# jdhuang-csm/hybrid-drt

Measured on AMD Instinct MI355X. Metric: DRT fits/sec (256 freq x 512 tau, batched), higher is better.
Workload: dtype f64

## Files before the change

hybrid-drt_amd/csrc/gram.hip:

```cpp
#include "common.hpp"
#include <type_traits>

namespace hipdrt {

typedef double v4d __attribute__((ext_vector_type(4)));

static constexpr int GT = 64;
static constexpr int GK = 16;
static constexpr int GLD = 80;


__host__ __device__ inline bool gram_strip_folds(int n) { const int nt16 = (n + 15) >> 4; return (nt16 & 3) == 1 && nt16 > 1; }

struct GramSub { int r, c; };
__host__ __device__ constexpr GramSub gram_diag_sub(int e) {
    const int r = e >= 10 ? 4 : e >= 6 ? 3 : e >= 3 ? 2 : e >= 1 ? 1 : 0;
    return GramSub{r, e >= 14 ? 4 : e >= 10 ? e - 10 : e - r * (r + 1) / 2};
}

template <int TURN>
__device__ __forceinline__ void gram_diag_slab(const double* sl, v4d (&acc)[4], int needm) {
#pragma unroll
    for (int kk = 0; kk < GK; kk += 4) {
        double x[5];
#pragma unroll
        for (int c = 0; c < 5; ++c) x[c] = sl[kk * GLD + c * 16];
#pragma unroll
        for (int s = 0; s < 4; ++s) {
            const GramSub sub = gram_diag_sub(TURN + 4 * s);
            if (needm & (1 << s)) acc[s] = __builtin_amdgcn_mfma_f64_16x16x4f64(x[sub.c], x[sub.r], acc[s], 0, 0, 0);
        }
    }
}

template <bool DOP, bool ROWP>
__global__ __launch_bounds__(256, 5) void gram_kernel(int m, int n, const double* __restrict__ A, int lda,
                                                   const double* __restrict__ w, GramL2 g, double* __restrict__ P,
                                                   int ldp, long long p_stride, const int* __restrict__ active,
                                                   int ntile, double* __restrict__ Ppk, long long ppk_stride, int nchp,
                                                   long long a_stride) {
    const int b = blockIdx.y;
    if (active && !active[b]) return;
    A += (size_t)b * a_stride;
    int t = blockIdx.x, ti = 0;
    while (t >= ti + 1) { t -= ti + 1; ++ti; }
    const int tj = t;
    const int i0 = ti * GT, j0 = tj * GT;
    const bool diag = (ti == tj);
    const int nt16 = (n + 15) >> 4;
    const bool strip = diag && gram_strip_folds(n);
    const int s0 = (nt16 - 1) * 16;
    const bool last = strip && i0 + GT == s0;

    __shared__ double sI[GK * GLD];
    __shared__ double sJ[GK * GLD];

    const int tid = threadIdx.x, lane = tid & 63, wv = __builtin_amdgcn_readfirstlane(tid >> 6);
    const double* wb = w + (size_t)b * m;
    double* Pk = Ppk ? Ppk + (size_t)b * ppk_stride : nullptr;

    int nown = 0, needm = 0;
    const int turn = (wv + 2 * (ti & 1)) & 3;
    if (diag) {
        const int rows_all = (Pk && nchp > nt16 ? nchp : nt16) - 4 * ti, rows_data = nt16 - 4 * ti;
        const int nr = rows_all < 4 ? rows_all : 4, nd = rows_data < 4 ? rows_data : 4;
        nown = nr * (nr + 1) / 2 + (strip ? 4 : 0) + (last ? 1 : 0);
        const int nneed = strip ? nown : nd * (nd + 1) / 2;
#pragma unroll
        for (int s = 0; s < 4; ++s) needm |= (turn + 4 * s < nneed) << s;
    }
    const int qr = 4 * ti + 2 * (wv >> 1), qc = 4 * tj + 2 * (wv & 1);
    const bool need00 = qr < nt16 && qc < nt16, need01 = qr < nt16 && qc + 1 < nt16;
    const bool need10 = qr + 1 < nt16 && qc < nt16, need11 = qr + 1 < nt16 && qc + 1 < nt16;

    v4d acc[4];
#pragma unroll
    for (int s = 0; s < 4; ++s) acc[s] = (v4d){0.0, 0.0, 0.0, 0.0};

    const int sk = tid >> 4, sc = (tid & 15) * 4;
    const bool vec2 = ((lda | n) & 1) == 0 && (reinterpret_cast<size_t>(A) & 15) == 0;
    const bool full = vec2 && m >= GK && (m & (GK - 1)) == 0 && i0 + GT <= n && (diag || j0 + GT <= n);
    const bool smask = strip && s0 + (tid & 15) < n;
    double vi[4], vj[4], wkr = 0.0;
    const double *pI = nullptr, *pJ = nullptr;
    auto fetch = [&](auto DIAG, auto FORM, int k0) {
        constexpr bool D = decltype(DIAG)::value;
        constexpr int F = decltype(FORM)::value;
        if constexpr (F == 0) {
            wkr = wb[k0 + sk];
            const double2 t0 = *reinterpret_cast<const double2*>(pI), t1 = *reinterpret_cast<const double2*>(pI + 2);
            vi[0] = t0.x; vi[1] = t0.y; vi[2] = t1.x; vi[3] = t1.y;
            if constexpr (!D) {
                const double2 u0 = *reinterpret_cast<const double2*>(pJ), u1 = *reinterpret_cast<const double2*>(pJ + 2);
                vj[0] = u0.x; vj[1] = u0.y; vj[2] = u1.x; vj[3] = u1.y;
            } else if (strip) {
                vj[0] = *pJ;
            }
            pI += (size_t)GK * lda;
            pJ += (size_t)GK * lda;
        } else {
            const int k = k0 + sk;
#pragma unroll
            for (int e = 0; e < 4; ++e) { vi[e] = 0.0; vj[e] = 0.0; }
            wkr = 0.0;
            if (k < m) {
                wkr = wb[k];
                const double* row = A + (size_t)k * lda;
                if constexpr (F == 1) {
#pragma unroll
                    for (int e = 0; e < 4; e += 2) {
                        const int ci = i0 + sc + e, cj = j0 + sc + e;
                        if (ci < n) { const double2 t = *reinterpret_cast<const double2*>(row + ci); vi[e] = t.x; vi[e + 1] = t.y; }
                        if (!D && cj < n) { const double2 t = *reinterpret_cast<const double2*>(row + cj); vj[e] = t.x; vj[e + 1] = t.y; }
                    }
                } else {
#pragma unroll
                    for (int e = 0; e < 4; ++e) {
                        const int ci = i0 + sc + e, cj = j0 + sc + e;
                        if (ci < n) vi[e] = row[ci];
                        if (!D && cj < n) vj[e] = row[cj];
                    }
                }
                if (D && smask) vj[0] = row[s0 + (tid & 15)];
            }
        }
    };
    auto kloop = [&](auto DIAG, auto TURN, auto FORM) {
        constexpr bool D = decltype(DIAG)::value;
        constexpr bool FULL = decltype(FORM)::value == 0;
        if constexpr (FULL) {
            pI = A + (size_t)sk * lda + i0 + sc;
            pJ = A + (size_t)sk * lda + (D ? (smask ? s0 + (tid & 15) : n - 1) : j0 + sc);
        }
        fetch(DIAG, FORM, 0);
        for (int k0 = 0; k0 < m; k0 += GK) {
            __syncthreads();
            *reinterpret_cast<double2*>(&sI[sk * GLD + sc]) = make_double2(wkr * vi[0], wkr * vi[1]);
            *reinterpret_cast<double2*>(&sI[sk * GLD + sc + 2]) = make_double2(wkr * vi[2], wkr * vi[3]);
            if (!D) {
                *reinterpret_cast<double2*>(&sJ[sk * GLD + sc]) = make_double2(wkr * vj[0], wkr * vj[1]);
                *reinterpret_cast<double2*>(&sJ[sk * GLD + sc + 2]) = make_double2(wkr * vj[2], wkr * vj[3]);
            } else if (strip) {
                sI[sk * GLD + GT + (tid & 15)] = wkr * (FULL && !smask ? 0.0 : vj[0]);
            }
            __syncthreads();
            if (k0 + GK < m) fetch(DIAG, FORM, k0 + GK);
            if (!D) {
                const int wi = (wv >> 1) * 32, wj = (wv & 1) * 32;
#pragma unroll
                for (int kk = 0; kk < GK; kk += 4) {
                    const int kr = kk + (lane >> 4);
                    double a0 = sI[kr * GLD + wi + (lane & 15)];
                    double a1 = sI[kr * GLD + wi + 16 + (lane & 15)];
                    double b0 = sJ[kr * GLD + wj + (lane & 15)];
                    double b1 = sJ[kr * GLD + wj + 16 + (lane & 15)];
                    if (FULL || need00) acc[0] = __builtin_amdgcn_mfma_f64_16x16x4f64(b0, a0, acc[0], 0, 0, 0);
                    if (FULL || need01) acc[1] = __builtin_amdgcn_mfma_f64_16x16x4f64(b1, a0, acc[1], 0, 0, 0);
                    if (FULL || need10) acc[2] = __builtin_amdgcn_mfma_f64_16x16x4f64(b0, a1, acc[2], 0, 0, 0);
                    if (FULL || need11) acc[3] = __builtin_amdgcn_mfma_f64_16x16x4f64(b1, a1, acc[3], 0, 0, 0);
                }
            } else {
                const double* sl = sI + (lane >> 4) * GLD + (lane & 15);
                gram_diag_slab<decltype(TURN)::value>(sl, acc, needm);
            }
        }
    };
    auto kform = [&](auto DIAG, auto TURN) {
        if (full) kloop(DIAG, TURN, std::integral_constant<int, 0>{});
        else if (vec2) kloop(DIAG, TURN, std::integral_constant<int, 1>{});
        else kloop(DIAG, TURN, std::integral_constant<int, 2>{});
    };
    if (!diag) kform(std::false_type{}, std::integral_constant<int, 0>{});
    else if (turn == 0) kform(std::true_type{}, std::integral_constant<int, 0>{});
    else if (turn == 1) kform(std::true_type{}, std::integral_constant<int, 1>{});
    else if (turn == 2) kform(std::true_type{}, std::integral_constant<int, 2>{});
    else kform(std::true_type{}, std::integral_constant<int, 3>{});

    double* sqI = sI;
    double* sqJ = sJ;
    constexpr int TW = 2 * GT;
    double* tw = sI + 3 * GT;
    const int dbase = i0 - j0 - (GT - 1);
    constexpr int SW = GT + 16;
    double* sqS = sJ + 3 * GT;
    double* tws = sJ + 4 * GT;
    const int dbase_s = s0 - j0 - (GT - 1);
    double fac[3] = {0, 0, 0};
    const bool reach_known = !DOP && g.toep && g.toep_maxd >= 0 && (j0 >= g.ns || g.spec_zero);
    const bool l2on = g.s && !(reach_known && i0 >= g.ns && dbase > g.toep_maxd);
    const bool l2on_s = strip && g.s && !(reach_known && s0 >= g.ns && dbase_s > g.toep_maxd);
    if (l2on) {
#pragma unroll
        for (int k = 0; k < 3; ++k) fac[k] = g.dfac[k] * (g.use_rho ? g.rho[(size_t)b * 3 + k] : 1.0);
        __syncthreads();
        const double* sb_ = g.s + (size_t)b * 3 * n;
        for (int e = tid; e < 3 * GT; e += 256) {
            const int k = e / GT, c = e % GT;
            sqI[e] = (i0 + c < n) ? sqrt(sb_[k * n + i0 + c]) : 0.0;
            sqJ[e] = (j0 + c < n) ? sqrt(sb_[k * n + j0 + c]) : 0.0;
        }
        if (strip && tid < 3 * 16) {
            const int k = tid >> 4, c = tid & 15;
            sqS[tid] = (s0 + c < n) ? sqrt(sb_[k * n + s0 + c]) : 0.0;
        }
        if (g.toep) {
            const int nd = n - g.ns;
            for (int e = tid; e < 3 * TW; e += 256) {
                const int k = e / TW, sl = e % TW;
                int dd = dbase + sl;
                dd = dd < 0 ? -dd : dd;
                tw[e] = (g.dfac[k] > 0.0 && dd < nd) ? g.mk[k][(size_t)g.ns * g.ldm + g.ns + dd] * fac[k] : 0.0;
            }
            if (l2on_s && tid < 3 * SW) {
                const int k = tid / SW, dd = dbase_s + tid % SW;
                tws[tid] = (g.dfac[k] > 0.0 && dd < nd) ? g.mk[k][(size_t)g.ns * g.ldm + g.ns + dd] * fac[k] : 0.0;
            }
        }
        __syncthreads();
    }
    double* Pb = (ROWP && P) ? P + (size_t)b * p_stride : nullptr;
    double dfac2[3] = {0, 0, 0};
    if (l2on) {
        if (DOP) {
#pragma unroll
            for (int k = 0; k < 3; ++k) dfac2[k] = g.dop_dfac[k] * (g.use_rho ? g.dop_rho[(size_t)b * 3 + k] : 1.0);
        }
    }
    const int dop_lo = DOP ? g.dop_start : 0, dop_hi = DOP ? g.dop_start + g.dop_size : 0;
#pragma unroll
    for (int s = 0; s < 4; ++s) {
        int r16 = qr + (s >> 1), c16 = qc + (s & 1);
        bool srow = false, scol = false;
        if (diag) {
            const int e = turn + 4 * s;
            if (e >= nown) continue;
            const GramSub sub = gram_diag_sub(e);
            srow = sub.r == 4;
            scol = sub.c == 4;
            r16 = srow ? nt16 - 1 : 4 * ti + sub.r;
            c16 = scol ? nt16 - 1 : 4 * ti + sub.c;
        }
        const bool sw = srow && !scol;
        const bool on = sw ? l2on_s : l2on;
        const double* sqr = srow ? sqS - s0 : sqI - i0;
        const double* sqc = scol ? sqS - s0 : sqJ - j0;
        const int rstr = srow ? 16 : GT, cstr = scol ? 16 : GT;
        const double* win = sw ? tws - dbase_s : tw - dbase;
        const int wstr = sw ? SW : TW;
        double vals[4];
#pragma unroll
        for (int r = 0; r < 4; ++r) {
            const int i = r16 * 16 + (lane & 15);
            const int j = c16 * 16 + (lane >> 4) + 4 * r;
            double v = 0.0;
            if (i < n && j < n) {
                v = acc[s][r];
                if (on) {
                    double l2 = 0.0;
#pragma unroll
                    for (int k = 0; k < 3; ++k) {
                        if (g.dfac[k] > 0.0) {
                            double mv;
                            if (g.toep && i >= g.ns && j >= g.ns) {
                                mv = win[k * wstr + (i - j)];
                            } else {
                                mv = g.sym ? g.mk[k][(size_t)j * g.ldm + i] : g.mk[k][(size_t)i * g.ldm + j];
                                if (i >= g.ns && j >= g.ns) mv *= fac[k];
                                else if (DOP && i >= dop_lo && i < dop_hi && j >= dop_lo && j < dop_hi) mv *= dfac2[k];
                            }
                            l2 += (sqr[k * rstr + i] * mv) * sqc[k * cstr + j];
                        }
                    }
                    v += l2;
                } else if (!g.s && g.l2) {
                    v += g.l2[(size_t)b * g.l2_stride + (size_t)i * g.ldl2 + j];
                }
                if (ROWP && Pb && j <= i) {
                    Pb[(size_t)i * ldp + j] = v;
                    if (i != j) Pb[(size_t)j * ldp + i] = v;
                }
            }
            vals[r] = v;
        }
        if (Pk && r16 < nchp && c16 < nchp && r16 >= c16) {
            double2* tile = reinterpret_cast<double2*>(Pk + ((size_t)r16 * nchp + c16) * 256);
            const int fo = (lane & 15) * 4 + (lane >> 4);
            tile[fo] = make_double2(vals[0], vals[1]);
            tile[64 + fo] = make_double2(vals[2], vals[3]);
        }
    }
    if (Pk && strip) {
        const int pe = nchp < nt16 + 3 ? nchp : nt16 + 3;
        for (int pr = nt16; pr < pe; ++pr) {
#pragma unroll
            for (int h = 0; h < 2; ++h) {
                const int pc = h ? nt16 - 1 + wv : 4 * ti + wv;
                if (h && !(last && pc <= pr)) continue;
                double2* tile = reinterpret_cast<double2*>(Pk + ((size_t)pr * nchp + pc) * 256);
                tile[lane] = make_double2(0.0, 0.0);
                tile[64 + lane] = make_double2(0.0, 0.0);
            }
        }
    }
}

__global__ __launch_bounds__(64) void pack_p_kernel(int n, const double* __restrict__ P, int ldp, long long p_stride,
                                                    double* __restrict__ Ppk, long long ppk_stride, int nchp) {
    int t = blockIdx.x, tr = 0;
    while (t >= tr + 1) { t -= tr + 1; ++tr; }
    const int tc = t, b = blockIdx.y, lane = threadIdx.x;
    const double* Pb = P + (size_t)b * p_stride;
    double vals[4];
#pragma unroll
    for (int r = 0; r < 4; ++r) {
        const int i = tr * 16 + (lane & 15), j = tc * 16 + (lane >> 4) + 4 * r;
        double v = 0.0;
        if (i < n && j < n) v = (i >= j) ? Pb[(size_t)i * ldp + j] : Pb[(size_t)j * ldp + i];
        vals[r] = v;
    }
    double2* tile = reinterpret_cast<double2*>(Ppk + (size_t)b * ppk_stride + ((size_t)tr * nchp + tc) * 256);
    const int fo = (lane & 15) * 4 + (lane >> 4);
    tile[fo] = make_double2(vals[0], vals[1]);
    tile[64 + fo] = make_double2(vals[2], vals[3]);
}

__global__ __launch_bounds__(256) void qvec_kernel(int m, int n, const double* __restrict__ A, int lda,
                                                   const double* __restrict__ w, const double* __restrict__ y,
                                                   const double* __restrict__ l1, double l1_scalar,
                                                   double* __restrict__ q, const int* __restrict__ active,
                                                   long long a_stride) {
    const int b = blockIdx.y;
    if (active && !active[b]) return;
    A += (size_t)b * a_stride;
    __shared__ double sw[256], swy[256];
    const int i = blockIdx.x * 256 + threadIdx.x;
    const double* wb = w + (size_t)b * m;
    const double* yb = y + (size_t)b * m;
    double acc = 0.0;
    for (int k0 = 0; k0 < m; k0 += 256) {
        __syncthreads();
        const int kk = k0 + threadIdx.x;
        if (kk < m) { const double wk = wb[kk]; sw[threadIdx.x] = wk; swy[threadIdx.x] = wk * yb[kk]; }
        __syncthreads();
        const int lim = (m - k0) < 256 ? (m - k0) : 256;
        if (i < n) {
            for (int k = 0; k < lim; ++k) acc += (sw[k] * A[(size_t)(k0 + k) * lda + i]) * swy[k];
        }
    }
    if (i < n) q[(size_t)b * n + i] = -acc + (l1 ? l1[i] : l1_scalar);
}

__global__ __launch_bounds__(64) void pack_rows_kernel(int nrow, int ncol, int col_offset, const double* __restrict__ M,
                                                       int ldm, double* __restrict__ tiles, int nchp) {
    const int tr = blockIdx.y, tc = blockIdx.x, lane = threadIdx.x;
    double vals[4];
#pragma unroll
    for (int r = 0; r < 4; ++r) {
        const int i = tr * 16 + (lane & 15), j = tc * 16 + (lane >> 4) + 4 * r - col_offset;
        vals[r] = (i < nrow && j >= 0 && j < ncol) ? M[(size_t)i * ldm + j] : 0.0;
    }
    double2* tile = reinterpret_cast<double2*>(tiles + ((size_t)tr * nchp + tc) * 256);
    const int fo = (lane & 15) * 4 + (lane >> 4);
    tile[fo] = make_double2(vals[0], vals[1]);
    tile[64 + fo] = make_double2(vals[2], vals[3]);
}

void launch_pack_rows(hipStream_t st, int nrow, int ncol, int col_offset, const double* M, int ldm, int ntile_rows,
                      double* tiles, int nchp) {
    hipLaunchKernelGGL(pack_rows_kernel, dim3(nchp, ntile_rows), dim3(64), 0, st, nrow, ncol, col_offset, M, ldm, tiles,
                       nchp);
}

__global__ __launch_bounds__(256) void rows_outer_kernel(const double* __restrict__ Y, int nch, int ncol, int nrow, double scale,
                                                         double* __restrict__ out, int ld) {
    const int ti = blockIdx.y, tj = blockIdx.x;
    if (tj > ti) return;
    __shared__ double A[256], Bt[256];
    const int t = threadIdx.x, i = t >> 4, j = t & 15;
    auto at = [](int r, int k) { return 2 * ((k >> 3) * 64 + r * 4 + (k & 3)) + ((k >> 2) & 1); };
    double acc = 0.0;
    for (int c = 0; c < ncol; ++c) {
        A[t] = Y[((size_t)ti * nch + c) * 256 + t];
        Bt[t] = Y[((size_t)tj * nch + c) * 256 + t];
        __syncthreads();
#pragma unroll
        for (int k = 0; k < 16; ++k) acc += A[at(i, k)] * Bt[at(j, k)];
        __syncthreads();
    }
    const int r = ti * 16 + i, cc = tj * 16 + j;
    if (r < nrow && cc < nrow) {
        out[(size_t)r * ld + cc] = acc * scale;
        out[(size_t)cc * ld + r] = acc * scale;
    }
}

void launch_rows_outer(hipStream_t st, const double* Y, int nch, int ncol, int nex, int nrow, double scale, double* out, int ld) {
    hipLaunchKernelGGL(rows_outer_kernel, dim3(nex, nex), dim3(256), 0, st, Y, nch, ncol, nrow, scale, out, ld);
}

void launch_pack_p(hipStream_t st, int B, int n, const double* P, int ldp, long long p_stride, double* Ppk,
                   long long ppk_stride, int nchp) {
    const int nt = (n + 15) / 16;
    hipLaunchKernelGGL(pack_p_kernel, dim3(nt * (nt + 1) / 2, B), dim3(64), 0, st, n, P, ldp, p_stride, Ppk, ppk_stride,
                       nchp);
}

void launch_gram_l2(hipStream_t st, int B, int m, int n, const double* A, int lda, const double* w, const GramL2& g,
                    double* P, int ldp, long long p_stride, const int* active, double* Ppk, long long ppk_stride,
                    int nchp, long long a_stride) {
    const int nt = gram_strip_folds(n) ? ((n + 15) / 16) / 4 : (n + GT - 1) / GT;
    const int ntile = nt * (nt + 1) / 2;
    const bool dop = g.s && g.dop_size > 0;
#define HIPDRT_GRAM(D, R) hipLaunchKernelGGL((gram_kernel<D, R>), dim3(ntile, B), dim3(256), 0, st, m, n, A, lda, w, g, P, ldp, \
                                             p_stride, active, ntile, Ppk, ppk_stride, nchp, a_stride)
    if (P) { if (dop) HIPDRT_GRAM(true, true); else HIPDRT_GRAM(false, true); }
    else { if (dop) HIPDRT_GRAM(true, false); else HIPDRT_GRAM(false, false); }
#undef HIPDRT_GRAM
}

void launch_qvec(hipStream_t st, int B, int m, int n, const double* A, int lda, const double* w, const double* y,
                 const double* l1, double l1_scalar, double* q, const int* active, long long a_stride) {
    if (a_stride == 0 && (size_t)m * n < ((size_t)1 << 20)) {
        launch_qvec_batched(st, B, m, n, A, lda, w, y, l1, l1_scalar, q, active);
        return;
    }
    hipLaunchKernelGGL(qvec_kernel, dim3((n + 255) / 256, B), dim3(256), 0, st, m, n, A, lda, w, y, l1, l1_scalar, q,
                       active, a_stride);
}

void launch_weighted_gram(hipStream_t st, int B, int m, int n, const double* A, int lda, const double* w,
                          const double* b, const double* l2, long long l2_stride, int ldl2, const double* l1,
                          double* P, int ldp, long long p_stride, double* q, const int* active) {
    GramL2 g{};
    g.l2 = l2; g.l2_stride = l2_stride; g.ldl2 = ldl2; g.s = nullptr;
    launch_gram_l2(st, B, m, n, A, lda, w, g, P, ldp, p_stride, active);
    launch_qvec(st, B, m, n, A, lda, w, b, l1, 0.0, q, active);
}

}
```

Baseline: 2745.

## Double-buffer half-slab K loop in gram kernel with one barrier per step

Replaces the full-tile K loop of the Gram kernel with a double-buffered scheme over half-slabs of 8 rows. Each step reads LDS operands, stages the next half-slab into the other buffer, issues the global prefetch and then the MFMAs, so only one __syncthreads is needed per step instead of two. The aim is to hide barrier and LDS-store latency behind MFMA work. The cost is more complex scheduling via sched_barrier and a changed thread-to-data mapping; the full path now also accepts m that is a multiple of 8.

```diff
diff --git a/hybrid-drt_amd/csrc/gram.hip b/hybrid-drt_amd/csrc/gram.hip
--- a/hybrid-drt_amd/csrc/gram.hip
+++ b/hybrid-drt_amd/csrc/gram.hip
@@ -7,6 +7,7 @@
 
 static constexpr int GT = 64;
 static constexpr int GK = 16;
+static constexpr int GH = GK / 2;
 static constexpr int GLD = 80;
 
 
@@ -18,18 +19,25 @@
     return GramSub{r, e >= 14 ? 4 : e >= 10 ? e - 10 : e - r * (r + 1) / 2};
 }
 
+__device__ __forceinline__ void gram_diag_read(const double* sl, double (&x)[5]) {
+#pragma unroll
+    for (int c = 0; c < 5; ++c) x[c] = sl[c * 16];
+}
+template <int TURN>
+__device__ __forceinline__ void gram_diag_mfma(const double (&x)[5], v4d (&acc)[4], int needm) {
+#pragma unroll
+    for (int s = 0; s < 4; ++s) {
+        const GramSub sub = gram_diag_sub(TURN + 4 * s);
+        if (needm & (1 << s)) acc[s] = __builtin_amdgcn_mfma_f64_16x16x4f64(x[sub.c], x[sub.r], acc[s], 0, 0, 0);
+    }
+}
 template <int TURN>
 __device__ __forceinline__ void gram_diag_slab(const double* sl, v4d (&acc)[4], int needm) {
 #pragma unroll
     for (int kk = 0; kk < GK; kk += 4) {
         double x[5];
-#pragma unroll
-        for (int c = 0; c < 5; ++c) x[c] = sl[kk * GLD + c * 16];
-#pragma unroll
-        for (int s = 0; s < 4; ++s) {
-            const GramSub sub = gram_diag_sub(TURN + 4 * s);
-            if (needm & (1 << s)) acc[s] = __builtin_amdgcn_mfma_f64_16x16x4f64(x[sub.c], x[sub.r], acc[s], 0, 0, 0);
-        }
+        gram_diag_read(sl + kk * GLD, x);
+        gram_diag_mfma<TURN>(x, acc, needm);
     }
 }
 
@@ -77,61 +85,110 @@
 #pragma unroll
     for (int s = 0; s < 4; ++s) acc[s] = (v4d){0.0, 0.0, 0.0, 0.0};
 
+    const bool vec2 = ((lda | n) & 1) == 0 && (reinterpret_cast<size_t>(A) & 15) == 0;
+    const bool full = vec2 && m >= GH && (m & (GH - 1)) == 0 && i0 + GT <= n && (diag || j0 + GT <= n);
+
+    auto kloop_full = [&](auto DIAG, auto TURN) {
+        constexpr bool D = decltype(DIAG)::value;
+        const int hk = tid >> 5, hs = tid & 31, hc = hs * 2;
+        const bool sown = strip && hs < 16;
+        const bool smask = sown && s0 + hs < n;
+        const double* pI = A + (size_t)hk * lda + i0 + hc;
+        const double* pJ = A + (size_t)hk * lda + (D ? (smask ? s0 + hs : n - 1) : j0 + hc);
+        const double* pw = wb + hk;
+        double2 ui, uj = make_double2(0.0, 0.0);
+        double wk;
+        auto fetch = [&]() {
+            wk = *pw;
+            ui = *reinterpret_cast<const double2*>(pI);
+            if constexpr (!D) uj = *reinterpret_cast<const double2*>(pJ);
+            else if (strip) uj.x = *pJ;
+            pw += GH;
+            pI += (size_t)GH * lda;
+            pJ += (size_t)GH * lda;
+        };
+        auto stage = [&](int half) {
+            *reinterpret_cast<double2*>(&sI[half + hk * GLD + hc]) = make_double2(wk * ui.x, wk * ui.y);
+            if constexpr (!D) *reinterpret_cast<double2*>(&sJ[half + hk * GLD + hc]) = make_double2(wk * uj.x, wk * uj.y);
+            else if (sown) sI[half + hk * GLD + GT + hs] = wk * (smask ? uj.x : 0.0);
+        };
+        const double* oI = sI + (lane >> 4) * GLD + (lane & 15) + (D ? 0 : (wv >> 1) * 32);
+        const double* oJ = sJ + (lane >> 4) * GLD + (lane & 15) + (wv & 1) * 32;
+        auto turn_of = [&](int cur, int nxt, bool next, bool ahead) {
+            static_assert(GH == 8, "a half-slab is two MFMA k-steps");
+            if constexpr (!D) {
+                double a0 = oI[cur], a1 = oI[cur + 16], b0 = oJ[cur], b1 = oJ[cur + 16];
+                if (next) stage(nxt);
+                __builtin_amdgcn_sched_barrier(0);
+                if (ahead) fetch();
+                acc[0] = __builtin_amdgcn_mfma_f64_16x16x4f64(b0, a0, acc[0], 0, 0, 0);
+                acc[1] = __builtin_amdgcn_mfma_f64_16x16x4f64(b1, a0, acc[1], 0, 0, 0);
+                acc[2] = __builtin_amdgcn_mfma_f64_16x16x4f64(b0, a1, acc[2], 0, 0, 0);
+                acc[3] = __builtin_amdgcn_mfma_f64_16x16x4f64(b1, a1, acc[3], 0, 0, 0);
+                a0 = oI[cur + 4 * GLD]; a1 = oI[cur + 4 * GLD + 16]; b0 = oJ[cur + 4 * GLD]; b1 = oJ[cur + 4 * GLD + 16];
+                acc[0] = __builtin_amdgcn_mfma_f64_16x16x4f64(b0, a0, acc[0], 0, 0, 0);
+                acc[1] = __builtin_amdgcn_mfma_f64_16x16x4f64(b1, a0, acc[1], 0, 0, 0);
+                acc[2] = __builtin_amdgcn_mfma_f64_16x16x4f64(b0, a1, acc[2], 0, 0, 0);
+                acc[3] = __builtin_amdgcn_mfma_f64_16x16x4f64(b1, a1, acc[3], 0, 0, 0);
+            } else {
+                double x[5];
+                gram_diag_read(oI + cur, x);
+                if (next) stage(nxt);
+                __builtin_amdgcn_sched_barrier(0);
+                if (ahead) fetch();
+                gram_diag_mfma<decltype(TURN)::value>(x, acc, needm);
+                gram_diag_read(oI + cur + 4 * GLD, x);
+                gram_diag_mfma<decltype(TURN)::value>(x, acc, needm);
+            }
+            if (next) __syncthreads();
+        };
+        const int nh = m / GH;
+        fetch();
+        stage(0);
+        if (nh > 1) fetch();
+        __syncthreads();
+        int h = 0;
+        for (; h + 3 < nh; h += 2) {
+            turn_of(0, GH * GLD, true, true);
+            turn_of(GH * GLD, 0, true, true);
+        }
+        for (; h < nh; ++h)
+            turn_of((h & 1) * GH * GLD, (~h & 1) * GH * GLD, h + 1 < nh, h + 2 < nh);
+    };
+
     const int sk = tid >> 4, sc = (tid & 15) * 4;
-    const bool vec2 = ((lda | n) & 1) == 0 && (reinterpret_cast<size_t>(A) & 15) == 0;
-    const bool full = vec2 && m >= GK && (m & (GK - 1)) == 0 && i0 + GT <= n && (diag || j0 + GT <= n);
     const bool smask = strip && s0 + (tid & 15) < n;
     double vi[4], vj[4], wkr = 0.0;
-    const double *pI = nullptr, *pJ = nullptr;
     auto fetch = [&](auto DIAG, auto FORM, int k0) {
         constexpr bool D = decltype(DIAG)::value;
         constexpr int F = decltype(FORM)::value;
-        if constexpr (F == 0) {
-            wkr = wb[k0 + sk];
-            const double2 t0 = *reinterpret_cast<const double2*>(pI), t1 = *reinterpret_cast<const double2*>(pI + 2);
-            vi[0] = t0.x; vi[1] = t0.y; vi[2] = t1.x; vi[3] = t1.y;
-            if constexpr (!D) {
-                const double2 u0 = *reinterpret_cast<const double2*>(pJ), u1 = *reinterpret_cast<const double2*>(pJ + 2);
-                vj[0] = u0.x; vj[1] = u0.y; vj[2] = u1.x; vj[3] = u1.y;
-            } else if (strip) {
-                vj[0] = *pJ;
-            }
-            pI += (size_t)GK * lda;
-            pJ += (size_t)GK * lda;
-        } else {
-            const int k = k0 + sk;
-#pragma unroll
-            for (int e = 0; e < 4; ++e) { vi[e] = 0.0; vj[e] = 0.0; }
-            wkr = 0.0;
-            if (k < m) {
-                wkr = wb[k];
-                const double* row = A + (size_t)k * lda;
-                if constexpr (F == 1) {
-#pragma unroll
-                    for (int e = 0; e < 4; e += 2) {
-                        const int ci = i0 + sc + e, cj = j0 + sc + e;
-                        if (ci < n) { const double2 t = *reinterpret_cast<const double2*>(row + ci); vi[e] = t.x; vi[e + 1] = t.y; }
-                        if (!D && cj < n) { const double2 t = *reinterpret_cast<const double2*>(row + cj); vj[e] = t.x; vj[e + 1] = t.y; }
-                    }
-                } else {
-#pragma unroll
-                    for (int e = 0; e < 4; ++e) {
-                        const int ci = i0 + sc + e, cj = j0 + sc + e;
-                        if (ci < n) vi[e] = row[ci];
-                        if (!D && cj < n) vj[e] = row[cj];
-                    }
+        const int k = k0 + sk;
+#pragma unroll
+        for (int e = 0; e < 4; ++e) { vi[e] = 0.0; vj[e] = 0.0; }
+        wkr = 0.0;
+        if (k < m) {
+            wkr = wb[k];
+            const double* row = A + (size_t)k * lda;
+            if constexpr (F == 1) {
+#pragma unroll
+                for (int e = 0; e < 4; e += 2) {
+                    const int ci = i0 + sc + e, cj = j0 + sc + e;
+                    if (ci < n) { const double2 t = *reinterpret_cast<const double2*>(row + ci); vi[e] = t.x; vi[e + 1] = t.y; }
+                    if (!D && cj < n) { const double2 t = *reinterpret_cast<const double2*>(row + cj); vj[e] = t.x; vj[e + 1] = t.y; }
                 }
-                if (D && smask) vj[0] = row[s0 + (tid & 15)];
-            }
+            } else {
+#pragma unroll
+                for (int e = 0; e < 4; ++e) {
+                    const int ci = i0 + sc + e, cj = j0 + sc + e;
+                    if (ci < n) vi[e] = row[ci];
+                    if (!D && cj < n) vj[e] = row[cj];
+                }
+            }
+            if (D && smask) vj[0] = row[s0 + (tid & 15)];
         }
     };
     auto kloop = [&](auto DIAG, auto TURN, auto FORM) {
         constexpr bool D = decltype(DIAG)::value;
-        constexpr bool FULL = decltype(FORM)::value == 0;
-        if constexpr (FULL) {
-            pI = A + (size_t)sk * lda + i0 + sc;
-            pJ = A + (size_t)sk * lda + (D ? (smask ? s0 + (tid & 15) : n - 1) : j0 + sc);
-        }
         fetch(DIAG, FORM, 0);
         for (int k0 = 0; k0 < m; k0 += GK) {
             __syncthreads();
@@ -141,7 +198,7 @@
                 *reinterpret_cast<double2*>(&sJ[sk * GLD + sc]) = make_double2(wkr * vj[0], wkr * vj[1]);
                 *reinterpret_cast<double2*>(&sJ[sk * GLD + sc + 2]) = make_double2(wkr * vj[2], wkr * vj[3]);
             } else if (strip) {
-                sI[sk * GLD + GT + (tid & 15)] = wkr * (FULL && !smask ? 0.0 : vj[0]);
+                sI[sk * GLD + GT + (tid & 15)] = wkr * vj[0];
             }
             __syncthreads();
             if (k0 + GK < m) fetch(DIAG, FORM, k0 + GK);
@@ -154,10 +211,10 @@
                     double a1 = sI[kr * GLD + wi + 16 + (lane & 15)];
                     double b0 = sJ[kr * GLD + wj + (lane & 15)];
                     double b1 = sJ[kr * GLD + wj + 16 + (lane & 15)];
-                    if (FULL || need00) acc[0] = __builtin_amdgcn_mfma_f64_16x16x4f64(b0, a0, acc[0], 0, 0, 0);
-                    if (FULL || need01) acc[1] = __builtin_amdgcn_mfma_f64_16x16x4f64(b1, a0, acc[1], 0, 0, 0);
-                    if (FULL || need10) acc[2] = __builtin_amdgcn_mfma_f64_16x16x4f64(b0, a1, acc[2], 0, 0, 0);
-                    if (FULL || need11) acc[3] = __builtin_amdgcn_mfma_f64_16x16x4f64(b1, a1, acc[3], 0, 0, 0);
+                    if (need00) acc[0] = __builtin_amdgcn_mfma_f64_16x16x4f64(b0, a0, acc[0], 0, 0, 0);
+                    if (need01) acc[1] = __builtin_amdgcn_mfma_f64_16x16x4f64(b1, a0, acc[1], 0, 0, 0);
+                    if (need10) acc[2] = __builtin_amdgcn_mfma_f64_16x16x4f64(b0, a1, acc[2], 0, 0, 0);
+                    if (need11) acc[3] = __builtin_amdgcn_mfma_f64_16x16x4f64(b1, a1, acc[3], 0, 0, 0);
                 }
             } else {
                 const double* sl = sI + (lane >> 4) * GLD + (lane & 15);
@@ -166,7 +223,7 @@
         }
     };
     auto kform = [&](auto DIAG, auto TURN) {
-        if (full) kloop(DIAG, TURN, std::integral_constant<int, 0>{});
+        if (full) kloop_full(DIAG, TURN);
         else if (vec2) kloop(DIAG, TURN, std::integral_constant<int, 1>{});
         else kloop(DIAG, TURN, std::integral_constant<int, 2>{});
     };
```

After: 2759, median of 6. About the same (+0.5%).
